# ckonst/VNDecorrelate

Hardware: AMD Instinct MI355X
Metric: Msamples/sec decorrelated (stereo, 30 taps) + achieved HBM GB/s vs roofline (higher is better)
Workload: dtype f32

## Files before the change

### vndecorrelate_amd/csrc/vnd_win.hpp

```cpp
#pragma once
#include "vnd_spec.hpp"
#include <cmath>
#include <functional>

namespace vnd {

static const char kWinKernelSource[] =
#include "vnd_win_kernel.inc"
    ;

struct WinGeom {
    int M = 0, nt = 0, G = 8;
    int C = 2;
    int DE = 0;
    int R = 0;
    int NB = 0;
    int plane = 0;
    int npl = 2;
    int tail = 0;
    int quad = 0;
    int split = 0;
    int nh() const { return split ? nt / 2 : (quad ? nt / (4 * quad) : nt); }
    int quad_pad() const { return quad == 2 ? 16 : 0; }
    size_t lds_bytes() const { return (size_t)(quad ? 2 * quad : 1) * (size_t)npl * (size_t)(M / 4) * (size_t)plane + (size_t)quad_pad(); }
// ... 76 lines not shown
                    if (j >= 1 && j <= M - 3) rd.ops.push_back(WinOp{1, (j - 1) / 2, h, tp.second, i});
                    else if (j == -1) rd.ops.push_back(WinOp{2, 0, h, tp.second, i});
                    else if (j == M - 1) rd.ops.push_back(WinOp{3, 0, h, tp.second, i});
                }
            }
        }
        if (!rd.ops.empty()) out.push_back(std::move(rd));
    }
    return out;
}

inline void win_traffic(const SpecTable &t, int M, size_t *lds_bytes, size_t *fmas)
{
    *lds_bytes = 0; *fmas = 0;
    for (int ch = 0; ch < t.C; ++ch) {
        *lds_bytes += 16 * win_schedule(t, ch, M).size();
        for (int32_t k = t.tap_off[ch]; k < t.tap_off[ch + 1]; ++k) if (t.w[k] != 0.0f) *fmas += (size_t)M;
    }
}

inline std::string win_taps_name(int pg) { return pg == 0 ? std::string("vw_taps") : "vw_taps_" + std::to_string(pg); }

inline std::string win_taps_channel_name(int pg, int ch)
{
    return pg == 0 ? "vw_taps_c" + std::to_string(ch) : "vw_taps_" + std::to_string(pg) + "c" + std::to_string(ch);
}

inline std::string win_taps_dispatch(const SpecTable &t)
{
    std::string s = "template <int PG> __device__ __forceinline__ void vw_taps_of(vw_lchar *const (&b)[2][VW_NBT], float (&o0)[VW_M], float (&o1)[VW_M])\n{\n";
    for (int pg = 0; pg < t.C / 2; ++pg)
        spec_append(s, "    %sif constexpr (PG == %d) %s(b, o0, o1);\n", pg ? "else " : "", pg, win_taps_name(pg).c_str());
    s += "}\n#define VW_DISPATCH(pg) switch (pg) {";
    for (int pg = 0; pg < t.C / 2; ++pg) spec_append(s, " case %d: vw_span<%d>(a, lds, stream, t_first, ntiles, flags, pace); break;", pg, pg);
    s += " default: break; }\n";
    return s;
}

inline std::string win_rd(const WinGeom &g, int ch, int o)
{
    const int dE = o / g.M, rr = (o % g.M) / 4;
    const int first_tail = g.R - g.nh() + 1;
    char buf[96];
    if (g.tail > 0 && dE >= first_tail) snprintf(buf, sizeof buf, "VW_RD(b[%d][%d], %d)", ch, g.NB + (dE - first_tail), rr * g.plane);
    else { const int kb = dE / g.G; snprintf(buf, sizeof buf, "VW_RD(b[%d][%d], %d)", ch, kb, (dE - kb * g.G) * 16 + rr * g.plane); }
    return buf;
}

inline bool win_adds_ok(const SpecTable &t)
{
    std::vector<float> mags;
    for (size_t k = 0; k < t.w.size(); ++k) {
        const float m = std::fabs(t.w[k]);
        if (m == 0.0f) continue;
        if (!std::isfinite(m) || m < 1e-18f || m > 1e18f) return false;
        if (std::find(mags.begin(), mags.end(), m) == mags.end()) mags.push_back(m);
        if (mags.size() > 8) return false;
    }
    for (int ch = 0; ch < t.C; ++ch) {
        std::vector<std::pair<int, float>> taps;
        for (int32_t k = t.tap_off[ch]; k < t.tap_off[ch + 1]; ++k)
            if (t.w[k] != 0.0f) taps.push_back({t.idx[k], std::fabs(t.w[k])});
        std::stable_sort(taps.begin(), taps.end(), [](const std::pair<int, float> &a, const std::pair<int, float> &b) { return a.first < b.first; });
        int changes = 0;
        for (size_t k = 1; k < taps.size(); ++k) changes += taps[k].second != taps[k - 1].second;
        if (changes > 8) return false;
    }
    return !mags.empty();
}

inline float win_unit_ratio(float from, float to) { return (float)((double)from / (double)to); }

inline void win_emit_adds_op(std::string &s, const std::string &acc, const std::string &x, bool pair, float w, float *unit)
{
    const float mag = std::fabs(w);
    const char sign = std::signbit(w) ? '-' : '+';
    if (*unit == 0.0f) spec_append(s, "    %s = %s %c %s;\n", acc.c_str(), pair ? "Z2" : "0.0f", sign, x.c_str());
    else if (*unit == mag) spec_append(s, "    %s = %s %c %s;\n", acc.c_str(), acc.c_str(), sign, x.c_str());
    else spec_append(s, "    %s = %s(%s, %s, %s%s);\n", acc.c_str(), pair ? "VW_FMA" : "__builtin_fmaf", acc.c_str(), spec_float(win_unit_ratio(*unit, mag)).c_str(),
                     sign == '-' ? "-" : "", x.c_str());
    *unit = mag;
}

template <class Name>
inline void win_emit_adds_merge(std::string &s, int ch, int M, const std::vector<float> &e_unit, const std::vector<float> &p_unit, float o0_unit, float ol_unit, Name name)
{
    float common = 0.0f;
    bool uniform = true;
    auto see = [&](float u) { if (u == 0.0f) return; if (common == 0.0f) common = u; else if (u != common) uniform = false; };
    for (float u : e_unit) see(u);
    for (float u : p_unit) see(u);
    see(o0_unit); see(ol_unit);
    for (int j = 0; j < M; ++j) {
        const float eu = e_unit[j / 2];
        const float ou = j == 0 ? o0_unit : (j == M - 1 ? ol_unit : p_unit[(j - 1) / 2]);
        std::string ev = eu != 0.0f ? (name(0, j / 2) + "." + ((j & 1) ? "y" : "x")) : std::string();
        std::string ov;
        if (ou != 0.0f) ov = j == 0 ? name(2, 0) : (j == M - 1 ? name(3, 0) : name(1, (j - 1) / 2) + "." + ((j & 1) ? "x" : "y"));
        if (!uniform) {
            if (!ev.empty()) ev = "(" + ev + " * " + spec_float(eu) + ")";
            if (!ov.empty()) ov = "(" + ov + " * " + spec_float(ou) + ")";
        }
        const std::string rhs = ev.empty() ? (ov.empty() ? std::string("0.0f") : ov) : (ov.empty() ? ev : ev + " + " + ov);
        spec_append(s, "    o%d[%d] = %s;\n", ch, j, rhs.c_str());
    }
    if (uniform && common != 0.0f && common != 1.0f) {
        const std::string u = spec_float(common);
        for (int k = 0; k < M / 2; ++k)
            spec_append(s, "    { const v2f t2 = v2f{o%d[%d], o%d[%d]} * v2f{%s, %s}; o%d[%d] = t2.x; o%d[%d] = t2.y; }\n", ch, 2 * k, ch, 2 * k + 1, u.c_str(), u.c_str(),
                        ch, 2 * k, ch, 2 * k + 1);
    }
}

inline std::string win_taps_function(const SpecTable &t, const WinGeom &g, int la, int pg = 0, int only_ch = -1, bool adds = false)
{
    const int M = g.M;
    std::string s;
    const std::string fname = only_ch < 0 ? win_taps_name(pg) : win_taps_channel_name(pg, only_ch);
    s += "__device__ __forceinline__ void " + fname + "(vw_lchar *const (&b)[2][VW_NBT], float (&o0)[VW_M], float (&o1)[VW_M])\n{\n";
    spec_append(s, "    v4f q[%d];\n    v2f E[%d], P[%d];\n    float O0, OL;\n", la + 1, M / 2, M / 2);
    if (adds) s += "    const v2f Z2 = {0.0f, 0.0f};\n";
    std::vector<WinRead> reads;
    size_t first_of_ch[3] = {0, 0, 0};
    for (int ch = 0; ch < 2; ++ch) {
        first_of_ch[ch] = reads.size();
        if (only_ch >= 0 && ch != only_ch) continue;
        std::vector<WinRead> one = win_schedule(t, 2 * pg + ch, M);
        std::reverse(one.begin(), one.end());
        if (adds)
            for (WinRead &r : one) std::stable_sort(r.ops.begin(), r.ops.end(), [](const WinOp &a, const WinOp &b) { return a.tap > b.tap; });
        for (WinRead &r : one) { r.ch = ch; reads.push_back(std::move(r)); }
    }
    first_of_ch[2] = reads.size();
    auto emit_read = [&](size_t k) {
        const WinRead &r = reads[k];
        spec_append(s, "    q[%zu] = %s;\n", k % (size_t)(la + 1), win_rd(g, r.ch, r.o).c_str());
    };
    auto emit_merge = [&](int ch, const std::vector<char> &e_used, const std::vector<char> &p_used, bool o0_used, bool ol_used) {
        for (int j = 0; j < M; ++j) {
            std::string ev = e_used[j / 2] ? ("E[" + std::to_string(j / 2) + "]." + ((j & 1) ? "y" : "x")) : std::string();
            std::string ov;
            if (j == 0) { if (o0_used) ov = "O0"; }
            else if (j == M - 1) { if (ol_used) ov = "OL"; }
            else if (p_used[(j - 1) / 2]) ov = "P[" + std::to_string((j - 1) / 2) + "]." + ((j & 1) ? "x" : "y");
            std::string rhs = ev.empty() ? (ov.empty() ? std::string("0.0f") : ov) : (ov.empty() ? ev : ev + " + " + ov);
            spec_append(s, "    o%d[%d] = %s;\n", ch, j, rhs.c_str());
        }
    };
    for (size_t k = 0; k < std::min(reads.size(), (size_t)la); ++k) emit_read(k);
    for (int ch = 0; ch < 2; ++ch) {
        if (only_ch >= 0 && ch != only_ch) continue;
        std::vector<char> e_used(M / 2, 0), p_used(M / 2, 0);
        bool o0_used = false, ol_used = false;
        std::vector<float> e_unit(M / 2, 0.0f), p_unit(M / 2, 0.0f);
        float o0_unit = 0.0f, ol_unit = 0.0f;
        for (size_t k = first_of_ch[ch]; k < first_of_ch[ch + 1]; ++k) {
            if (k + la < reads.size()) emit_read(k + la);
            const std::string qk = "q[" + std::to_string(k % (size_t)(la + 1)) + "]";
            for (const WinOp &op : reads[k].ops) {
                const std::string w = spec_float(op.w);
                if (adds) {
                    const bool pair = op.kind <= 1, is0 = op.kind == 2;
                    const std::string acc = pair ? std::string(op.kind == 0 ? "E[" : "P[") + std::to_string(op.acc) + "]" : std::string(is0 ? "O0" : "OL");
                    const std::string x = pair ? qk + (op.half ? ".zw" : ".xy") : qk + (is0 ? (op.half ? ".w" : ".y") : (op.half ? ".z" : ".x"));
                    win_emit_adds_op(s, acc, x, pair, op.w, pair ? (op.kind == 0 ? &e_unit[op.acc] : &p_unit[op.acc]) : (is0 ? &o0_unit : &ol_unit));
                    continue;
                }
                if (op.kind <= 1) {
                    const std::string acc = std::string(op.kind == 0 ? "E[" : "P[") + std::to_string(op.acc) + "]";
                    const std::string x = qk + (op.half ? ".zw" : ".xy");
                    char &used = op.kind == 0 ? e_used[op.acc] : p_used[op.acc];
                    if (used) spec_append(s, "    %s = VW_FMA(%s, %s, %s);\n", acc.c_str(), x.c_str(), w.c_str(), acc.c_str());
                    else spec_append(s, "    %s = VW_MUL(%s, %s);\n", acc.c_str(), x.c_str(), w.c_str());
                    used = 1;
                } else {
                    const bool is0 = op.kind == 2;
                    const std::string acc = is0 ? "O0" : "OL";
                    const std::string x = qk + (is0 ? (op.half ? ".w" : ".y") : (op.half ? ".z" : ".x"));
                    bool &used = is0 ? o0_used : ol_used;
                    if (used) spec_append(s, "    %s = __builtin_fmaf(%s, %s, %s);\n", acc.c_str(), x.c_str(), w.c_str(), acc.c_str());
                    else spec_append(s, "    %s = %s * %s;\n", acc.c_str(), x.c_str(), w.c_str());
                    used = true;
                }
            }
            s += "    VW_SB;\n";
        }
        if (adds)
            win_emit_adds_merge(s, ch, M, e_unit, p_unit, o0_unit, ol_unit, [](int kind, int k) {
                return kind == 0 ? "E[" + std::to_string(k) + "]" : (kind == 1 ? "P[" + std::to_string(k) + "]" : std::string(kind == 2 ? "O0" : "OL"));
            });
        else emit_merge(ch, e_used, p_used, o0_used, ol_used);
    }
    s += "}\n";
    return s;
}

struct WinExTap { int idx; float w; };
struct WinExPass { int ch; std::vector<WinExTap> taps; int end; float gain; };
struct WinExOp { int type, k; float w; };
struct WinExRead { int ch, o; size_t pass; std::vector<WinExOp> ops; };

inline std::vector<WinExPass> win_exact_passes(const SpecTable &t, int ch)
{
    std::vector<WinExPass> out;
    const int32_t k0 = t.tap_off[ch], k1 = t.tap_off[ch + 1];
    if (k0 == k1) return out;
    auto add_segment = [&](int32_t a, int32_t b, int end, float gain) {
        int32_t start = a;
        for (int32_t k = a + 1; k <= b; ++k) {
            if (k == b || t.idx[k] < t.idx[k - 1]) {
                WinExPass ps{ch, {}, k == b ? end : 0, gain};
                for (int32_t m = start; m < k; ++m) ps.taps.push_back(WinExTap{t.idx[m], t.w_raw[m]});
                out.push_back(std::move(ps));
                start = k;
            }
        }
    };
    if (!t.has_seg) {
        add_segment(k0, k1, 1, 1.0f);
    } else {
        int32_t prev = k0;
        for (int32_t sg = t.seg_off[ch]; sg < t.seg_off[ch + 1]; ++sg) {
            add_segment(prev, t.seg_end[sg], t.apply_gain ? 3 : 2, t.seg_gain[sg]);
            prev = t.seg_end[sg];
        }
    }
    return out;
}

inline void win_exact_reads(const std::vector<WinExPass> &passes, int M, std::vector<WinExRead> *reads, size_t pass_base)
{
    for (size_t p = 0; p < passes.size(); ++p) {
        const WinExPass &ps = passes[p];
        std::map<int, std::vector<WinExOp>> by_chunk;
        const bool singles = true;
        for (const WinExTap &tp : ps.taps) {
            if (singles && (tp.idx & 1)) {
                for (int j = -1; j < M; j += 2) {
                    const int e = tp.idx + j;
                    by_chunk[(e & 3) == 0 ? e : e - 2].push_back(WinExOp{((e & 3) == 0 ? 0 : 1) | 4, j, tp.w});
                }
                continue;
            }
            for (int j = 0; j < M; j += 2) {
                const int e = tp.idx + j;
                switch (e & 3) {
                case 0: by_chunk[e].push_back(WinExOp{0, j / 2, tp.w}); break;
                case 2: by_chunk[e - 2].push_back(WinExOp{1, j / 2, tp.w}); break;
                case 1: by_chunk[e - 1].push_back(WinExOp{3, j / 2, tp.w}); break;
                default: by_chunk[e + 1].push_back(WinExOp{2, j / 2, tp.w}); break;
                }
            }
        }
        std::vector<int> lend;
        for (const auto &kv : by_chunk)
            for (const WinExOp &op : kv.second)
                if (op.type == 2) { lend.push_back(kv.first - 4); break; }
        for (int o : lend) by_chunk[o];
        for (auto &kv : by_chunk) reads->push_back(WinExRead{ps.ch, kv.first, pass_base + p, std::move(kv.second)});
    }
}

inline void win_traffic_exact(const SpecTable &t, int M, size_t *lds_bytes, size_t *fmas)
{
    *lds_bytes = 0; *fmas = 0;
    for (int ch = 0; ch < t.C; ++ch) {
        std::vector<WinExRead> reads;
        const std::vector<WinExPass> passes = win_exact_passes(t, ch);
        if (!passes.empty()) win_exact_reads(passes, M, &reads, 0);
        *lds_bytes += 16 * reads.size();
        *fmas += (size_t)M * (size_t)(t.tap_off[ch + 1] - t.tap_off[ch]);
    }
}
// ... 430 lines not shown
```

### vndecorrelate_amd/csrc/vnd_win_kernel.inc

```
R"VNDWIN(
// vnd_spec_kernel, WINDOW form - the per-table tap sum with a register window (gfx950, wave64).
//
// Compiled at run time with hipRTC (vnd_win.hpp) behind a generated prologue that defines
//   VW_NT   threads per workgroup                 VW_M   consecutive output frames a lane owns per tile (16 | 32 | 64)
//   VW_R    ring entries (one entry = the M frames of one lane's run): NT of the tile + VW_DE of halo
//   VW_G    entries mirrored behind the ring, = the reach of one base register
//   VW_NB   base registers per channel (VW_DE / VW_G + 1)
//   VW_PLANE  bytes between the LDS planes of consecutive 16-byte chunks of an entry
//   VW_LA   LDS reads kept in flight ahead of the FMAs
//   VW_C    interleaved channels of the signal (even): a workgroup takes ONE channel pair of a span, 8 bytes of
//           every VW_C*4-byte frame (VW_C = 2: the whole frame, 16-byte accesses)
//   VW_Q    1: the QUAD form for signals of 4k channels - a workgroup takes a channel QUAD of a span (16 bytes of every
//           frame), a wave computes ONE channel of it (tap functions vw_taps_<pair>c<channel>) and stages and stores whole
//           16-byte pieces for all four (vw_span_qc below)
//           2: the OCTET form for signals of 8k channels - two neighbouring quads (32 bytes of every frame: with 8 channels,
//           whole frames and whole cache lines) per workgroup, an eighth of its lanes per channel
//   VW_S    1: the SPLIT form of a stereo signal - half the workgroup's waves compute channel 0, the others channel 1 (the tap
//           functions vw_taps_c0 / vw_taps_c1): a lane carries one channel's accumulators, so three waves fit a SIMD's registers
//           where the plain form holds two (vw_span_s below)
// and the functions vw_taps(), vw_taps_1(), ... (at the marker below): the tap sum of ONE lane for each channel
// pair, fully unrolled, with vw_taps_of<PG>() to pick one and VW_DISPATCH(pg): the span loop vw_span<pg> of a run-time pair number.
//
// The reference's tap sum (decorrelation.py:649-658, :402-414) asks, per output sample, for one input sample
// per tap.  vnd_spec_kernel.inc reads each of them from LDS (one aligned ds_read_b64 per tap and output
// ... 49 lines not shown
    // CHUNK of chunk_tiles consecutive tiles of one stream; the one dispatched first takes chunk_len0 of them, the next the rest
    // (chunk_tiles == 0: uniform spans, units walked as above)
    int chunk_tiles, chunk_len0, chunks_per_stream, cus_per_xcd;
    int stagger_ticks;       // a CU's second workgroup starts its prologue this many 100 MHz ticks after it enters the kernel
    int chunk_prio;          // 1: a CU's first-dispatched workgroup (the longer piece: the launch's critical path) runs at raised wave priority
    // BALANCED cut (stereo, uniform spans that would fill the resident workgroups unevenly): bal_total = streams x tiles_total > 0 - logical
    // workgroup L of nblocks walks the pool's tiles [L * bal_total / nblocks, (L + 1) * bal_total / nblocks), stream by stream: every
    // workgroup the same number of tiles (+- 1), a range that crosses into the next stream pays one more ring fill
    int bal_total;
    // VW_EPI, 32-frame runs: a wave's 64 runs are one 2048-frame block of the exact RMS sums (vnd_epilogue.hpp, rms_par_*): its sums of
    // squares of x and of the finished y, [stream][x0 x1 y0 y1][block] - the float64 PREDICTIONS the block-parallel sums start from
    // (every step of those is verified against the running sum: the values need not be the reference's, only close)
    double *epi_blk_sum;
    int epi_nblocks;
    int epi_rows_major;      // 1: [stream][block][x0 x1 y0 y1] instead - the rows epilogue_reduce_kernel adds up (the fused fast stage)
    // PACING of a CU's two co-resident workgroups (one round of persistent workgroups): the SIMDs issue the OLDER wave first, so the
    // workgroup publishes its count of finished tiles in its CU's slot pair and reads its partner's: the one BEHIND runs its next tile at
    // raised wave priority.  pace: [CU index][2] counters in device memory (never reset: a stale count only costs the first tile its bias)
    unsigned *pace;
};

struct VWPace { unsigned *mine; const unsigned *other; unsigned done; };

constexpr int VW_NW = VW_NT / 64;
constexpr int VW_QC = VW_M / 4;                 // 16-byte chunks per entry and channel
constexpr int VW_NH = VW_S ? VW_NT / 2 : VW_Q ? VW_NT / (4 * VW_Q) : VW_NT;  // lanes - and ring entries of a tile - per channel pair
constexpr int VW_T = VW_NH * VW_M;              // frames per tile
constexpr int VW_LPE = VW_Q ? VW_M * VW_Q : VW_M / 2;  // lanes of a 1 KB global access that fall into one entry (a lane moves a frame pair; VW_Q: one frame of four channels)
constexpr int VW_EPI_N = 64 / VW_LPE;           // entries per 1 KB global access
constexpr int VW_NI = VW_M / 2;                 // 1 KB global accesses per wave and tile
constexpr int VW_NPL = 2;                       // plane sets in LDS: one per output channel (the store phase transposes both channels' runs through them)
constexpr int VW_NXP = (VW_BC && !VW_S) ? 1 : 2; // ... of them holding INPUT: a mono input is staged once for both outputs (in the split form into both sets)
constexpr int VW_CH = VW_QC * VW_PLANE;         // byte offset of channel 1's planes
constexpr int VW_CX = VW_BC ? 1 : VW_C;         // interleaved INPUT channels
// channel pairs (VW_Q: quads or octets): one per workgroup and span.  4k + 2 channels (6, 10, ...) as QUADS: k full quads and one more that
// starts at channel C - 4 - it overlaps its neighbour in one channel pair, which both workgroups compute and write with the same bits
// (a frame's 16 bytes per access instead of the pair form's 8, for (k + 1) / (k + 1/2) of the arithmetic)
constexpr int VW_PAIRS = VW_Q ? (VW_C + 4 * VW_Q - 1) / (4 * VW_Q) : VW_C / 2;
constexpr int VW_PAIRB = 2 * VW_CH;             // VW_Q: byte offset of the second pair's plane sets
constexpr int VW_QUADB = 2 * VW_PAIRB + VW_QUADPAD; // octets: ... of the second QUAD's (shifted by 16 bytes: the two quads of a frame - neighbouring lanes of the 4-byte staging accesses - in different banks)
static_assert(VW_C >= 2 && VW_C % 2 == 0 && (VW_C == 2 || !VW_BC) && (VW_C == 2 || VW_Q || !VW_EPI), "whole channel pairs; fan-out and fused pointwise steps are stereo (quads / octets: the normaliser's sums only)");
static_assert(VW_Q == 0 || VW_Q == 1 || VW_Q == 2, "pairs, quads or octets");
static_assert(!VW_S || (VW_C == 2 && !VW_Q && !VW_EPI && VW_NT % 128 == 0 && VW_M >= 16), "split form: a stereo table, whole waves per channel");
static_assert(!VW_Q || ((VW_C % (4 * VW_Q) == 0 || (VW_Q == 1 && VW_C % 4 == 2 && VW_C >= 6)) && VW_NT % (256 * VW_Q) == 0 && VW_M * VW_Q <= 64 && VW_M <= 32), "quad / octet form: whole channel quads (4k + 2 channels: the last quad overlaps), whole waves per channel");
static_assert(VW_M == 16 || VW_M == 32 || VW_M == 64, "run length");
constexpr int VW_NBT = VW_NB + VW_TAIL;          // base registers per channel: the ring's, then one per entry offset that reaches into the tail
static_assert(VW_NT % 64 == 0 && VW_R >= VW_NH && VW_R + VW_TAIL == VW_NH + VW_DE && (VW_TAIL == 0 || (VW_Q && VW_R % 16 == 0)), "ring (+ tail) = tile + halo");
static_assert(VW_NB * VW_G > VW_DE, "bases cover the halo");
static_assert((VW_PLANE / 16) >= VW_R + VW_G + VW_TAIL, "plane stride: room for ring + mirror (+ tail)");
static_assert((VW_QC - 1) * VW_PLANE + VW_G * 16 < 65536 && VW_CH < 65536, "ds offset field is 16 bits");
static_assert((VW_Q ? 2 * VW_Q : 1) * VW_NPL * VW_QC * VW_PLANE + VW_QUADPAD <= 160 * 1024 && VW_QUADPAD % 16 == 0, "LDS");

// Raw buffer descriptor (stride 0): num_records = bytes left in the stream, so loads past the end of
// the stream return 0 (the reference's dropped terms, decorrelation.py:656-658) and stores past it
// are discarded.  Built from kernel arguments, blockIdx and the tile counter only: lives in SGPRs.
__device__ __forceinline__ v4i vw_rsrc(const void *base, long long bytes)
{
    const long long cap = 0x7fffffff;
    const unsigned long long addr = (unsigned long long)base;
    v4i r;
    r.x = (int)(unsigned)addr;
    r.y = (int)((unsigned)(addr >> 32) & 0xffffu);
    r.z = (int)(bytes < 0 ? 0 : (bytes > cap ? cap : bytes));
    r.w = 0x00020000;
    return r;
}

// blocks b and b + 8 share an XCD (and its L2): give one XCD consecutive logical ids, so that neighbouring
// spans (whose halos overlap) share an L2
__device__ __forceinline__ unsigned vw_xcd_remap(unsigned b, unsigned nwg)
{
    const unsigned q = nwg >> 3, r = nwg & 7u, xcd = b & 7u;
    const unsigned start = xcd < r ? xcd * (q + 1) : r * (q + 1) + (xcd - r) * q;
    return start + (b >> 3);
}

// (a mod R) for a < 2R, without a comparison: a - R wraps past 2^32 when a < R
__device__ __forceinline__ unsigned vw_wrap(unsigned a)
{
    const unsigned b = a - (unsigned)VW_R;
    return a < b ? a : b;
}

// one frame pair as {f0.c0, f0.c1, f1.c0, f1.c1}; a mono input fills the slots of channel 0.  In a wider signal the
// descriptor starts at the workgroup's channel pair: its 8 bytes of frames 2*pair and 2*pair + 1
__device__ __forceinline__ v4f vw_load_pair(v4i rsrc, int pair)
{
    if constexpr (VW_BC) {
        const v2f a = vw_load2(rsrc, pair * 8, 0, VW_LOAD_AUX);
        return v4f{a.x, 0.0f, a.y, 0.0f};
    } else if constexpr (VW_C == 2) {
        return vw_load4(rsrc, pair * 16, 0, VW_LOAD_AUX);
    } else {
        const v2f a = vw_load2(rsrc, pair * (VW_C * 8), 0, VW_LOAD_AUX), b = vw_load2(rsrc, pair * (VW_C * 8) + VW_C * 4, 0, VW_LOAD_AUX);
        return v4f{a.x, a.y, b.x, b.y};
    }
}

__device__ __forceinline__ void vw_store_pair(v4f v, v4i rsrc, int pair, int aux)
{
    if constexpr (VW_C == 2) {
        vw_store4(v, rsrc, pair * 16, 0, aux);
    } else {
        vw_store2(v2f{v.x, v.y}, rsrc, pair * (VW_C * 8), 0, aux);
        vw_store2(v2f{v.z, v.w}, rsrc, pair * (VW_C * 8) + VW_C * 4, 0, aux);
    }
}

// the staged pair goes to the channel planes (de-interleaved): 8 bytes each at `at` (chunk plane + entry + half)
__device__ __forceinline__ void vw_write_pair(vw_lchar *at, v4f v)
{
    *(vw_lv2f *)at = v2f{v.x, v.z};
    if constexpr (!VW_BC) *(vw_lv2f *)(at + VW_CH) = v2f{v.y, v.w};
}

#define VW_RD(base, imm) (*(const volatile vw_lv4f *)((base) + (imm)))
#define VW_FMA(x, w, a) __builtin_elementwise_fma((x), v2f{(w), (w)}, (a))
#define VW_MUL(x, w) ((x) * v2f{(w), (w)})
#define VW_SB __builtin_amdgcn_sched_barrier(0)
__device__ __forceinline__ float vw_add1(float a, float b)
{
    float r;
    asm("v_add_f32 %0, %1, %2" : "=v"(r) : "v"(a), "v"(b));
    return r;
}
__device__ __forceinline__ float vw_sub1(float a, float b)
{
    float r;
    asm("v_sub_f32 %0, %1, %2" : "=v"(r) : "v"(a), "v"(b));
    return r;
}
// (a.y, b.x) in ONE instruction: the exact mode's input pairs that start at an odd element (hipcc often takes two v_mov_b32)
__device__ __forceinline__ v2f vw_pair(v2f a, v2f b)
{
    v2f r;
    asm("v_pk_mov_b32 %0, %1, %2 op_sel:[1,0]" : "=v"(r) : "v"(a), "v"(b));
    return r;
}

//@@VW_TAPS@@

#if VW_STAMPS
// diagnosis (VND_WIN_STAMPS under VND_TUNING; tools/win_stamps.py): wave 0 of the first VW_STAMPS workgroups leaves the 100 MHz
// wall clock at its phase boundaries (first unit only) - [0] start, [1] ring filled, then for each of the first two tiles: taps done,
// (window dead: not kept), outputs exchanged, refill published; [14] the wave's stores acknowledged; [15] = HW_ID | XCC_ID << 32.  The stamps wait in SGPRs until the span is done
// (the kernel lives within a few VGPRs of its budget: a store per stamp made hipRTC's build spill).
__device__ unsigned long long vw_stamps[VW_STAMPS * 16];
#if VW_STAMP_PHASES
#define VW_STAMP_DECL unsigned vw_st[12] = {0, 0, 0, 0, 0, 0, 0, 0, 0, 0, 0, 0}
#define VW_STAMP(k) do { vw_st[k] = (unsigned)__builtin_amdgcn_s_memrealtime(); } while (0)
// ([12] = the workgroup's entry into the kernel, [13] = its exit (stores acknowledged), both written by the kernel function:
//  with VW_STAMP_PHASES 0 these two are all there is, and nothing is held in registers across the span)
#define VW_STAMP_FLUSH(on) do { if (on) { asm volatile("s_waitcnt vmcnt(0)" ::: "memory"); const unsigned long long end_ = __builtin_amdgcn_s_memrealtime(); if (threadIdx.x == VW_STAMP_WAVE * 64) { _Pragma("unroll") for (int q_ = 0; q_ < 12; ++q_) vw_stamps[blockIdx.x * 16 + q_] = vw_st[q_] ? (end_ - (unsigned long long)((unsigned)end_ - vw_st[q_])) : 0ull; vw_stamps[blockIdx.x * 16 + 14] = end_; } } } while (0)
#define VW_STAMP_TILE(t, k) do { if ((k) != 1 || VW_Q) { const unsigned now_ = (unsigned)__builtin_amdgcn_s_memrealtime(); _Pragma("unroll") for (int q_ = 0; q_ < 2; ++q_) if ((t) == q_) vw_st[2 + 4 * q_ + (k)] = now_; } } while (0)
#endif
#endif
#if !VW_STAMPS || !VW_STAMP_PHASES
#define VW_STAMP_DECL
#define VW_STAMP(k)
#define VW_STAMP_TILE(t, k)
#define VW_STAMP_FLUSH(on)
#endif

#if VW_EPI
// VelvetNoise.decorrelate's pointwise steps on one stereo frame, in the reference's float32 operation order
// (utils/dsp.py:59-63 side-channel encode, :34-37 stereo width; built with -ffp-contract=off)
__device__ __forceinline__ v2f vw_pointwise1(const VWArgs &a, v2f y, v2f x)          // one frame: {L, R}
{
    float y0 = y.x, y1 = y.y;
    if (a.epi_ms_encode) {
        const float mid = x.x + x.y;
        const float side = (y0 - y1) * 0.5f;
        y0 = (mid + side) * 0.5f;
        y1 = (mid - side) * 0.5f;
    }
    if (a.epi_use_width) {
        float m = (y0 + y1) * 0.5f, sd = (y0 - y1) * 0.5f;
        m = m * a.epi_w_mid;
        sd = sd * a.epi_w_side;
        y0 = m + sd;
        y1 = m - sd;
    }
    return v2f{y0, y1};
}
#endif

template <int PG>
__device__ __forceinline__ void vw_span(const VWArgs &a, vw_lchar *lds, long long stream, int t_first, int ntiles, int flags, VWPace &pace)
{
    const int tid = threadIdx.x;
    const int ln = tid & 63;
    const int wv = __builtin_amdgcn_readfirstlane(tid >> 6);
    const long long f0 = (long long)t_first * VW_T;
    // (the descriptors start at the channel pair: PGX / PG * 8 bytes into the first frame, and end as much before
    //  the end of the stream's last frame - inside the pair's last 8 bytes' frame, never in the next stream)
    constexpr int PGX = VW_BC ? 0 : PG;
// ... 397 lines not shown
        // With ONE wave per channel (NWH == 1: octets of 512 lanes, quads of 256) nobody else reads the channel's planes: the wave that
        // read the window is the one that overwrites it, in LDS program order - no barrier here, two per tile instead of three.
        if constexpr (NWH > 1) asm volatile("s_waitcnt lgkmcnt(0)\n\ts_barrier" ::: "memory");
        __builtin_amdgcn_s_setprio(1);
        vw_lchar *const mine = lp + (pc & 1) * VW_CH + pl * 16u;
#pragma unroll
        for (int r = 0; r < VW_QC; ++r)
            *(vw_lv4f *)(mine + r * VW_PLANE) = v4f{o[4 * r], o[4 * r + 1], o[4 * r + 2], o[4 * r + 3]};
        // X2. ... and the partner waves' (the other channels of the same 64 entries)
        asm volatile("s_waitcnt lgkmcnt(0)\n\ts_barrier" ::: "memory");
        VW_STAMP_TILE(t, 2);
        const long long fo = (long long)t * VW_T + (long long)we * VW_M;
        const v4i ry = vw_rsrc(ys + fo * VW_C, bytes_left - fo * FB);
        const long long fi = ((long long)(t + 1) * VW_NH + VW_R + we) * VW_M;
        const v4i rx = vw_rsrc(xs + fi * VW_C, bytes_need - fi * FB);
        constexpr int ST_AUX = VW_NT_STORES ? VW_NT_STORE_AUX : 0;
#pragma unroll
        for (int m = 0; m < NI; ++m) {
            vw_lchar *at = lds + lane_at + vw_wrap(pwl + (unsigned)(m * VW_EPI_N)) * 16u;
            const float c0 = *(const volatile vw_lfloat *)at, c1 = *(const volatile vw_lfloat *)(at + VW_CH);
            const float c2 = *(const volatile vw_lfloat *)(at + VW_PAIRB), c3 = *(const volatile vw_lfloat *)(at + VW_PAIRB + VW_CH);
            vw_store4(v4f{c0, c1, c2, c3}, ry, lg + m * (FPA * FB), 0, ST_AUX);
        }
        VW_STAMP_TILE(t, 1);                                                          // (quads / octets: read-backs and stores issued)
        const bool fin = (flags & 1) != 0 && t == ntiles - 1;          // (as vw_span: nothing to refill, nobody to wait for)
        if (!fin) {
            const bool mirror = pw < (unsigned)VW_G || pw + (unsigned)WE > (unsigned)VW_R;    // wave-uniform
#pragma unroll
            for (int m = 0; m < NI; ++m) {
                const unsigned e = vw_wrap(pwl + (unsigned)(m * VW_EPI_N));
                vw_lchar *at = lds + lane_at + e * 16u;
                vw_write_quad(at, pre[m]);
                if (mirror) { if (e < (unsigned)VW_G) vw_write_quad(at + VW_R * 16, pre[m]); }
                pre[m] = vw_load4(rx, lg + m * (FPA * FB), 0, VW_LOAD_AUX);
            }
#if VW_TAIL
            if (wv < NTA) {                                                              // wave-uniform
                const unsigned e = (unsigned)(wv * VW_EPI_N) + (unsigned)lane_e;
                if (e < (unsigned)VW_TAIL) vw_write_quad(lds + lane_at + ((unsigned)(VW_R + VW_G) + e) * 16u, tailreg);      // tile t + 1's
                const long long ft = ((long long)(t + 2) * VW_NH + VW_R + wv * VW_EPI_N) * VW_M;                               // tile t + 2's
                tailreg = vw_load4(vw_rsrc(xs + ft * VW_C, bytes_need - ft * FB), lg, 0, VW_LOAD_AUX);
            }
#endif
        }
        p0 = p0 + VW_NH >= VW_R ? p0 + VW_NH - VW_R : p0 + VW_NH;
        __builtin_amdgcn_s_setprio(0);
        if (!fin) asm volatile("s_waitcnt lgkmcnt(0)\n\ts_barrier" ::: "memory");
        VW_STAMP_TILE(t, 3);
    }
    VW_STAMP_FLUSH(vw_stamp_on);
}
#endif

#if VW_S
// ---- the SPLIT form of a stereo signal: a wave computes ONE channel ---------------------------------------
// The plain form's lane carries both channels' work one after the other: E / P accumulators, the first channel's finished
// outputs and a tile of prefetched frames - ~240 registers, two waves per SIMD.  Here waves 0 .. NW/2-1 run channel 0's tap
// function (vw_taps_c0) on the tile's NT/2 entries and the other half channel 1's: per lane one channel's accumulators, half
// the prefetch - three waves per SIMD fit (two workgroups of 384 lanes per CU: 12 waves), on the same ring and the same
// 1 KB global accesses.  A frame's two channels now sit in two waves: outputs go as planar runs into the tile's dead
// entries, one barrier more, then each wave reads back and stores the 32 entries it also refills (as vw_span_qc).
template <int CH>
__device__ __forceinline__ void vw_taps_ch(vw_lchar *const (&b)[2][VW_NBT], float (&o)[VW_M])
{
    if constexpr (CH == 0) vw_taps_c0(b, o, o);
    else vw_taps_c1(b, o, o);
}

__device__ __forceinline__ void vw_span_s(const VWArgs &a, vw_lchar *lds, long long stream, int t_first, int ntiles, int flags, VWPace &pace)
{
    constexpr int NWH = VW_NW / 2;                                       // waves per channel
    constexpr int NI = VW_M / 4;                                         // 1 KB global STORES per wave and tile (64 frame pairs each)
    // VW_BC - a mono input fanned out: the one input channel is staged into BOTH plane sets (each output channel's waves read their own
    // copy with the tap functions of the stereo form unchanged), 16 bytes = 4 frames per lane and access: half as many input accesses,
    // each 256 frames = 256 / M ring entries (stereo: 128 frames)
    constexpr int NIN = VW_BC ? VW_M / 8 : VW_M / 4;                     // 1 KB global LOADS per wave and tile
    constexpr int EIN = VW_BC ? 256 / VW_M : VW_EPI_N;                   // ring entries per load
    constexpr int XB = VW_BC ? 4 : 8;                                    // input bytes per frame
    // the refill's frames: NE accesses are prefetched a tile ahead and held in registers through the tap phase, the other
    // LATE are loaded at the start of the store phase that consumes them (64-frame runs: the accumulators need the room)
    constexpr int LATE = VW_LATE < NIN ? VW_LATE : NIN - 1;
    constexpr int NE = NIN - LATE;
    static_assert(VW_LATE >= 0 && LATE < NIN, "late refill accesses");
    const int tid = threadIdx.x;
    const int ln = tid & 63;
    const int wv = __builtin_amdgcn_readfirstlane(tid >> 6);
    const int pc = wv >= NWH ? 1 : 0;                                    // the wave's channel
    const int wl = wv - pc * NWH;
    const int tl = wl * 64 + ln;                                         // the entry of a tile this LANE computes (in its channel)
    const int we = wl * 64 + pc * 32;                                    // the first of the 32 entries this WAVE stages and stores (both channels)
    const long long f0 = (long long)t_first * VW_T;
    const float *xs = a.x + (stream * a.n + f0) * (XB / 4);
    float *ys = a.y + (stream * a.n + f0) * 2;
    const long long bytes_left = (a.n - f0) * 8;                         // (of the output)
    const long long need = ((long long)ntiles * VW_T + (long long)VW_DE * VW_M) * XB;
    const long long bytes_need = need < (a.n - f0) * XB ? need : (a.n - f0) * XB;
#if VW_LANE_SWIZZLE
    const int lq = (ln & ~24) | ((ln & 8) << 1) | ((ln & 16) >> 1);      // (as vw_span: the 8-byte staging writes and read-backs touch every bank once)
#else
    const int lq = ln;
#endif
    const int lane_e = lq / VW_LPE;
    const int lane_at = ((lq % VW_LPE) >> 1) * VW_PLANE + (lq & 1) * 8;
    // ... and in a 1 KB LOAD: stereo as above; mono - 4 frames = one 16-byte chunk of entry ln / (M / 4), written to both plane sets
    const int in_e = VW_BC ? ln / (VW_M / 4) : lane_e;
    const int in_at = VW_BC ? (ln % (VW_M / 4)) * VW_PLANE : lane_at;
    const int in16 = VW_BC ? ln * 16 : lq * 16;                          // the lane's byte offset in a load
    auto stage = [&](vw_lchar *at, v4f v) {
        if constexpr (VW_BC) { *(vw_lv4f *)at = v; *(vw_lv4f *)(at + VW_CH) = v; }
        else vw_write_pair(at, v);
    };
#if VW_STAMPS && VW_STAMP_PHASES
    const bool vw_stamp_on = blockIdx.x < VW_STAMPS && (a.chunk_tiles > 0 || a.bal_total > 0 || (unsigned)(stream * a.spans + t_first / a.tiles_per_span) == vw_xcd_remap(blockIdx.x, a.nblocks));
    if (vw_stamp_on && threadIdx.x == 0) {
        unsigned hw, xcc;
        asm volatile("s_getreg_b32 %0, hwreg(HW_REG_HW_ID)" : "=s"(hw));
        asm volatile("s_getreg_b32 %0, hwreg(HW_REG_XCC_ID)" : "=s"(xcc));
        vw_stamps[blockIdx.x * 16 + 15] = (unsigned long long)hw | ((unsigned long long)xcc << 32);
    }
#endif
    VW_STAMP_DECL;
    VW_STAMP(0);

    {
        const v4i rx = vw_rsrc(xs, bytes_need);
        constexpr int NFILL = (VW_R + EIN - 1) / EIN;
        constexpr int PER = (NFILL + VW_NW - 1) / VW_NW;
        constexpr int BATCH = 8;
        for (int k0 = 0; k0 < PER; k0 += BATCH) {
            v4f w[BATCH];
#pragma unroll
            for (int kk = 0; kk < BATCH; ++kk) {
                const int i = wv + VW_NW * (k0 + kk);
                w[kk] = vw_load4(rx, i * 1024 + in16, 0, VW_LOAD_AUX);
            }
#pragma unroll
            for (int kk = 0; kk < BATCH; ++kk) {
                const int i = wv + VW_NW * (k0 + kk);
                const int e = i * EIN + in_e;
                if (k0 + kk < PER && e < VW_R) {
                    stage(lds + in_at + e * 16, w[kk]);
                    if (e < VW_G) stage(lds + in_at + (e + VW_R) * 16, w[kk]);
                }
            }
        }
    }
    v4f pre[NE];
    {
        const long long f = ((long long)VW_R + we) * VW_M;
        const v4i rx = vw_rsrc(xs + f * (XB / 4), bytes_need - f * XB);
#pragma unroll
        for (int m = 0; m < NE; ++m) pre[m] = vw_load4(rx, 1024 * m + in16, 0, VW_LOAD_AUX);
    }
    asm volatile("s_waitcnt lgkmcnt(0)\n\ts_barrier" ::: "memory");
    VW_STAMP(1);
    bool hi = (flags & 2) != 0;                                          // (wave-uniform) raised priority: a chunk's first workgroup - or, paced, the one behind
    if (hi) __builtin_amdgcn_s_setprio(2);

    unsigned p0 = 0;
    for (int t = 0; t < ntiles; ++t) {
        // the last tile of the workgroup's last unit refills nothing: no loads, no staging writes, no barrier behind its stores
        const bool fin = (flags & 1) != 0 && t == ntiles - 1;
        const unsigned pw = vw_wrap(p0 + (unsigned)we);
        const unsigned pl = vw_wrap(p0 + (unsigned)tl);
        // (a lane's byte offset in a 1 KB access and its entry in it, made opaque per tile: hipcc otherwise hoists the sums with
        //  64-frame runs is what spilled)
        int lq16 = lq * 16, in16o = in16;
        unsigned pwl = pw + (unsigned)lane_e, pwi = pw + (unsigned)in_e;
        asm volatile("" : "+v"(lq16), "+v"(pwl));
        if constexpr (VW_BC) asm volatile("" : "+v"(in16o), "+v"(pwi));
        float o[VW_M];
        {
            vw_lchar *b[2][VW_NBT];
#pragma unroll
            for (int k = 0; k < VW_NB; ++k) {
                b[0][k] = lds + vw_wrap(pl + (unsigned)(k * VW_G)) * 16u;
                b[1][k] = b[0][k] + VW_CH;
            }
            if (pc == 0) vw_taps_ch<0>(b, o);
            else vw_taps_ch<1>(b, o);
        }
#pragma unroll
        for (int j = 0; j < VW_M; ++j) asm volatile("" : "+v"(o[j]));
        VW_STAMP_TILE(t, 0);
        // X. every wave is done reading this tile's window: the tile's own entries are dead (both channels)
        asm volatile("s_waitcnt lgkmcnt(0)\n\ts_barrier" ::: "memory");
        VW_STAMP_TILE(t, 1);
        if (hi) __builtin_amdgcn_s_setprio(3);
        else __builtin_amdgcn_s_setprio(1);
        // (pacing: the partner's count, in flight through the store phase)
        unsigned seen = 0;
        if (pace.other != nullptr) seen = __hip_atomic_load(pace.other, __ATOMIC_RELAXED, __HIP_MEMORY_SCOPE_AGENT);
        // (the late part of THIS tile's refill: in flight through the transposition and the stores)
        v4f late[LATE > 0 ? LATE : 1];
        if constexpr (LATE > 0) {                                        // (also on a final tile: out of range there, no data moves)
            const long long fl = ((long long)t * VW_NH + VW_R + we) * VW_M;
            const v4i rl = vw_rsrc(xs + fl * (XB / 4), bytes_need - fl * XB);
#pragma unroll
            for (int m = 0; m < LATE; ++m) late[m] = vw_load4(rl, (VW_BC ? in16o : lq16) + 1024 * (NE + m), 0, VW_LOAD_AUX);
        }
        // the lane's run into its own dead entry, planar (its channel's planes)
        vw_lchar *const mine = lds + pc * VW_CH + pl * 16u;
#pragma unroll
        for (int r = 0; r < VW_QC; ++r)
            *(vw_lv4f *)(mine + r * VW_PLANE) = v4f{o[4 * r], o[4 * r + 1], o[4 * r + 2], o[4 * r + 3]};
        // X2. ... and the partner wave's (the other channel of the same 64 entries)
        asm volatile("s_waitcnt lgkmcnt(0)\n\ts_barrier" ::: "memory");
        VW_STAMP_TILE(t, 2);
        const long long fo = (long long)t * VW_T + (long long)we * VW_M;
        const v4i ry = vw_rsrc(ys + fo * 2, bytes_left - fo * 8);
        const long long fi = ((long long)(t + 1) * VW_NH + VW_R + we) * VW_M;
        const v4i rx = vw_rsrc(xs + fi * (XB / 4), bytes_need - fi * XB);
        constexpr int ST_AUX = VW_NT_STORES ? VW_NT_STORE_AUX : 0;
        //  short launch nothing much, covers these round trips: tools/ablate/RUNS.md: run_r4c, run_r4g.sh)
#pragma unroll
        for (int m = 0; m < NI; ++m) {
            vw_lchar *at = lds + lane_at + vw_wrap(pwl + (unsigned)(m * VW_EPI_N)) * 16u;
            const v2f r0 = *(const volatile vw_lv2f *)at, r1 = *(const volatile vw_lv2f *)(at + VW_CH);
            vw_store4(v4f{r0.x, r1.x, r0.y, r1.y}, ry, lq16 + 1024 * m, 0, ST_AUX);
        }
        if (!fin) {
            const bool mirror = pw < (unsigned)VW_G || pw + 32u > (unsigned)VW_R;             // wave-uniform
#pragma unroll
            for (int m = 0; m < NIN; ++m) {
                const unsigned e = vw_wrap((VW_BC ? pwi : pwl) + (unsigned)(m * EIN));
                vw_lchar *at = lds + in_at + e * 16u;
                const v4f v = m < NE ? pre[m < NE ? m : 0] : late[m >= NE ? m - NE : 0];
                stage(at, v);
                if (mirror) { if (e < (unsigned)VW_G) stage(at + VW_R * 16, v); }
                if (m < NE) pre[m < NE ? m : 0] = vw_load4(rx, (VW_BC ? in16o : lq16) + 1024 * m, 0, VW_LOAD_AUX);
            }
        }
        p0 = p0 + VW_NH >= VW_R ? p0 + VW_NH - VW_R : p0 + VW_NH;
        pace.done += 1;
        if (pace.other != nullptr) {
            if (threadIdx.x == 0) __hip_atomic_store(pace.mine, pace.done, __ATOMIC_RELAXED, __HIP_MEMORY_SCOPE_AGENT);
            hi = (unsigned)__builtin_amdgcn_readfirstlane((int)seen) > pace.done;       // the partner is ahead: this workgroup's next tile goes first
        }
        if (hi) __builtin_amdgcn_s_setprio(2);
        else __builtin_amdgcn_s_setprio(0);
        // Y. the refill is in place for every wave's window
        if (!fin) asm volatile("s_waitcnt lgkmcnt(0)\n\ts_barrier" ::: "memory");
        VW_STAMP_TILE(t, 3);
    }
    if (hi) __builtin_amdgcn_s_setprio(0);
    VW_STAMP_FLUSH(vw_stamp_on);
}
#endif

// VW_WAVES_PER_EU: the waves per SIMD that the LDS footprint and the registers let a CU hold - as minimum AND maximum:
// the scheduler must not trade registers for an occupancy the LDS will not grant
extern "C" __global__ __launch_bounds__(VW_NT) __attribute__((amdgpu_waves_per_eu(VW_WAVES_PER_EU, VW_WAVES_PER_EU)))
void vnd_spec_kernel(const VWArgs a)
{
#if VW_STAMPS
    { const unsigned long long entry_ = __builtin_amdgcn_s_memrealtime(); if (threadIdx.x == 0 && blockIdx.x < VW_STAMPS) vw_stamps[blockIdx.x * 16 + 12] = entry_; }
#endif
    extern __shared__ __attribute__((aligned(16))) float lds_generic[];
    vw_lchar *lds = (vw_lchar *)(vw_lfloat *)lds_generic;
    // One round of workgroups: more units than resident slots are walked inside the kernel
    // (the channel pairs of a span are neighbouring units: their workgroups touch the same lines at about the same time)
    const unsigned first = vw_xcd_remap(blockIdx.x, a.nblocks);
    // (ONE call site of the span loop - it is the whole tap sum, inlined - for both ways of cutting the work)
    const bool chunked = VW_PAIRS == 1 && a.chunk_tiles > 0;
    VWPace pace = {nullptr, nullptr, 0u};
    if (a.pace != nullptr && !chunked) {
        // the CU this workgroup runs on (HW_ID: cu 11:8, sh 12, se 15:13; XCC_ID) and its dispatch round there
        unsigned hw, xcc;
        asm volatile("s_getreg_b32 %0, hwreg(HW_REG_HW_ID)" : "=s"(hw));
        asm volatile("s_getreg_b32 %0, hwreg(HW_REG_XCC_ID)" : "=s"(xcc));
        const unsigned cu = (((xcc & 7u) * 8u + ((hw >> 13) & 7u)) * 2u + ((hw >> 12) & 1u)) * 16u + ((hw >> 8) & 15u);
        const unsigned round = ((blockIdx.x >> 3) / (unsigned)a.cus_per_xcd) & 1u;
        pace.mine = a.pace + cu * 2u + round;
        pace.other = a.pace + cu * 2u + (round ^ 1u);
        if (threadIdx.x == 0) __hip_atomic_store(pace.mine, 0u, __ATOMIC_RELAXED, __HIP_MEMORY_SCOPE_AGENT);
    }
    const bool balanced = VW_PAIRS == 1 && !chunked && a.bal_total > 0;
    long long g = 0, g_end = 0;                                          // balanced: this workgroup's range of the pool's tiles
    if (balanced) {
        g = (long long)first * a.bal_total / (long long)a.nblocks;
        g_end = (long long)(first + 1u) * a.bal_total / (long long)a.nblocks;
    }
    for (unsigned unit = first; chunked || (balanced ? g < g_end : unit < a.units); unit += a.nblocks) {
        int pg = 0, t_first, ntiles;
        long long stream;
        if (balanced) {
            stream = g / a.tiles_total;
            t_first = (int)(g - stream * a.tiles_total);
            const long long left_s = a.tiles_total - t_first, left_w = g_end - g;
            ntiles = (int)(left_s < left_w ? left_s : left_w);
            g += ntiles;
        } else if (chunked) {
            // HW_ID, tools/win_stamps.py): workgroup j of XCD x runs on CU j mod cus_per_xcd as that CU's (j / cus_per_xcd)-th.  Were the
            // dispatch ever different, every piece would still be computed exactly once - only the balance would suffer.
            const unsigned xcd = blockIdx.x & 7u, j = blockIdx.x >> 3;
            const unsigned cu = j % (unsigned)a.cus_per_xcd, round = j / (unsigned)a.cus_per_xcd;
            const unsigned g = xcd * (unsigned)a.cus_per_xcd + cu;                           // the CU's chunk
            stream = g / (unsigned)a.chunks_per_stream;
            const int chunk = (int)(g % (unsigned)a.chunks_per_stream);
            const int len = round == 0 ? a.chunk_len0 : (round == 1 ? a.chunk_tiles - a.chunk_len0 : 0);
            t_first = chunk * a.chunk_tiles + (round == 0 ? 0 : a.chunk_len0);
            const int left = a.tiles_total - t_first;
            ntiles = left < len ? left : len;
            if (ntiles <= 0) break;
            if (round != 0 && a.stagger_ticks > 0) {
                const unsigned long long until = __builtin_amdgcn_s_memrealtime() + (unsigned long long)a.stagger_ticks;
                while (__builtin_amdgcn_s_memrealtime() < until) __builtin_amdgcn_s_sleep(8);
            }
        } else {
            unsigned id = unit;
            pg = (int)(id % (unsigned)VW_PAIRS);
            id /= (unsigned)VW_PAIRS;
// ... 18 lines not shown
```

Baseline: 698,600.

## Compute ring LDS addresses from wave-uniform parts and use packed moves for swizzles

Ring addresses for store and load accesses are now built from a wave-uniform first entry computed on the scalar unit plus one per-lane constant. This replaces per-lane wrap arithmetic, and the mirror test becomes scalar compares. Channel swizzles use v_pk_mov_b32 via inline asm instead of pairs of v_mov. Channel-1 LDS bases are made opaque so the compiler does not fold large offsets into each read. The aim is fewer VALU instructions per tile in the memory-bound store and refill phases. The cost is more complex edge-case logic at the ring end and the mirror region.

```diff
diff --git a/vndecorrelate_amd/csrc/vnd_win.hpp b/vndecorrelate_amd/csrc/vnd_win.hpp
--- a/vndecorrelate_amd/csrc/vnd_win.hpp
+++ b/vndecorrelate_amd/csrc/vnd_win.hpp
@@ -182,8 +182,13 @@
     *unit = mag;
 }
 
+inline std::string win_merge_sum(const std::string &ev, const std::string &ov, bool single)
+{
+    return single ? "vw_add1(" + ev + ", " + ov + ")" : ev + " + " + ov;
+}
+
 template <class Name>
-inline void win_emit_adds_merge(std::string &s, int ch, int M, const std::vector<float> &e_unit, const std::vector<float> &p_unit, float o0_unit, float ol_unit, Name name)
+inline void win_emit_adds_merge(std::string &s, int ch, int M, const std::vector<float> &e_unit, const std::vector<float> &p_unit, float o0_unit, float ol_unit, Name name, bool single = false)
 {
     float common = 0.0f;
     bool uniform = true;
@@ -201,7 +206,7 @@
             if (!ev.empty()) ev = "(" + ev + " * " + spec_float(eu) + ")";
             if (!ov.empty()) ov = "(" + ov + " * " + spec_float(ou) + ")";
         }
-        const std::string rhs = ev.empty() ? (ov.empty() ? std::string("0.0f") : ov) : (ov.empty() ? ev : ev + " + " + ov);
+        const std::string rhs = ev.empty() ? (ov.empty() ? std::string("0.0f") : ov) : (ov.empty() ? ev : win_merge_sum(ev, ov, single));
         spec_append(s, "    o%d[%d] = %s;\n", ch, j, rhs.c_str());
     }
     if (uniform && common != 0.0f && common != 1.0f) {
@@ -243,7 +248,7 @@
             if (j == 0) { if (o0_used) ov = "O0"; }
             else if (j == M - 1) { if (ol_used) ov = "OL"; }
             else if (p_used[(j - 1) / 2]) ov = "P[" + std::to_string((j - 1) / 2) + "]." + ((j & 1) ? "x" : "y");
-            std::string rhs = ev.empty() ? (ov.empty() ? std::string("0.0f") : ov) : (ov.empty() ? ev : ev + " + " + ov);
+            std::string rhs = ev.empty() ? (ov.empty() ? std::string("0.0f") : ov) : (ov.empty() ? ev : win_merge_sum(ev, ov, g.split != 0));
             spec_append(s, "    o%d[%d] = %s;\n", ch, j, rhs.c_str());
         }
     };
@@ -288,7 +293,7 @@
         if (adds)
             win_emit_adds_merge(s, ch, M, e_unit, p_unit, o0_unit, ol_unit, [](int kind, int k) {
                 return kind == 0 ? "E[" + std::to_string(k) + "]" : (kind == 1 ? "P[" + std::to_string(k) + "]" : std::string(kind == 2 ? "O0" : "OL"));
-            });
+            }, g.split != 0);
         else emit_merge(ch, e_used, p_used, o0_used, ol_used);
     }
     s += "}\n";
diff --git a/vndecorrelate_amd/csrc/vnd_win_kernel.inc b/vndecorrelate_amd/csrc/vnd_win_kernel.inc
--- a/vndecorrelate_amd/csrc/vnd_win_kernel.inc
+++ b/vndecorrelate_amd/csrc/vnd_win_kernel.inc
@@ -155,6 +155,25 @@
     return a < b ? a : b;
 }
 
+// instructions: written in C, hipcc spells either half with single v_mov_b32 - about six per 16-byte access of the store phase
+__device__ __forceinline__ v2f vw_lows(v2f a, v2f b)
+{
+    v2f r;
+    asm("v_pk_mov_b32 %0, %1, %2 op_sel:[0,0]" : "=v"(r) : "v"(a), "v"(b));
+    return r;
+}
+__device__ __forceinline__ v2f vw_highs(v2f a, v2f b)
+{
+    v2f r;
+    asm("v_pk_mov_b32 %0, %1, %2 op_sel:[1,1]" : "=v"(r) : "v"(a), "v"(b));
+    return r;
+}
+__device__ __forceinline__ v4f vw_zip(v2f a, v2f b)
+{
+    const v2f lo = vw_lows(a, b), hi = vw_highs(a, b);
+    return v4f{lo.x, lo.y, hi.x, hi.y};
+}
+
 // one frame pair as {f0.c0, f0.c1, f1.c0, f1.c1}; a mono input fills the slots of channel 0.  In a wider signal the
 // descriptor starts at the workgroup's channel pair: its 8 bytes of frames 2*pair and 2*pair + 1
 __device__ __forceinline__ v4f vw_load_pair(v4i rsrc, int pair)
@@ -183,8 +202,8 @@
 // the staged pair goes to the channel planes (de-interleaved): 8 bytes each at `at` (chunk plane + entry + half)
 __device__ __forceinline__ void vw_write_pair(vw_lchar *at, v4f v)
 {
-    *(vw_lv2f *)at = v2f{v.x, v.z};
-    if constexpr (!VW_BC) *(vw_lv2f *)(at + VW_CH) = v2f{v.y, v.w};
+    *(vw_lv2f *)at = vw_lows(v2f{v.x, v.y}, v2f{v.z, v.w});
+    if constexpr (!VW_BC) *(vw_lv2f *)(at + VW_CH) = vw_highs(v2f{v.x, v.y}, v2f{v.z, v.w});
 }
 
 #define VW_RD(base, imm) (*(const volatile vw_lv4f *)((base) + (imm)))
@@ -748,6 +767,20 @@
     constexpr int LATE = VW_LATE < NIN ? VW_LATE : NIN - 1;
     constexpr int NE = NIN - LATE;
     static_assert(VW_LATE >= 0 && LATE < NIN, "late refill accesses");
+    // RING ADDRESSES FROM WAVE-UNIFORM PARTS.  A wave's 32 entries start at pw, and access m of it takes the EPI_N (a store) or EIN (a
+    // load) entries from pw + m x that number on: the FIRST of them is wave-uniform - scalar arithmetic - and a lane adds ONE constant
+    // (its entry within the access, its chunk plane and half): one v_add_u32 per access.  That needs the entries of an access to stay
+    // together at the ring's end and at the mirror's:
+    //   * the ring's length and G multiples of their number - the ring advances by whole tiles (NH entries, a multiple of 64) and a wave
+    //     starts 32 entries into one, so every access then starts at a multiple too; or
+    //   * entry PAIRS (64-frame runs) on any ring: the pair that starts at the ring's last entry has its second half at entry 0 (the
+    //     lanes' other constant, picked by a scalar compare), and whether a lane's entry has a mirror - all of the pair below G - 1,
+    //     the first half at G - 1, the second at R - 1 - is a scalar compare and a fixed half of the wave.
+    // (Any other ring: per lane, as vw_span)
+    constexpr bool UNI_O = VW_EPI_N == 2 || VW_R % VW_EPI_N == 0;
+    constexpr bool UNI_I = EIN == 2 || (VW_R % EIN == 0 && VW_G % EIN == 0);
+    constexpr bool ENDS_O = VW_R % VW_EPI_N != 0, ENDS_I = VW_R % EIN != 0;      // an access can straddle the ring's end (pairs only)
+    static_assert(VW_NH % 64 == 0 && 32 % VW_EPI_N == 0 && 32 % EIN == 0, "a wave's accesses start at whole multiples of their entries");
     const int tid = threadIdx.x;
     const int ln = tid & 63;
     const int wv = __builtin_amdgcn_readfirstlane(tid >> 6);
@@ -772,9 +805,26 @@
     const int in_e = VW_BC ? ln / (VW_M / 4) : lane_e;
     const int in_at = VW_BC ? (ln % (VW_M / 4)) * VW_PLANE : lane_at;
     const int in16 = VW_BC ? ln * 16 : lq * 16;                          // the lane's byte offset in a load
+    // UNI_O / UNI_I: all of a lane's own in the LDS address of a store / load access, and (_w) where the access straddles the ring's end
+    int lane_c = lane_e * 16 + lane_at, lane_cw = lane_c - lane_e * (VW_R * 16), in_c = in_e * 16 + in_at, in_cw = in_c - in_e * (VW_R * 16);
+    asm volatile("" : "+v"(lane_c), "+v"(lane_cw));                      // (ONE register each: hipcc would take the sums apart again)
+    if constexpr (VW_BC) asm volatile("" : "+v"(in_c), "+v"(in_cw));
+    else { in_c = lane_c; in_cw = lane_cw; }
     auto stage = [&](vw_lchar *at, v4f v) {
         if constexpr (VW_BC) { *(vw_lv4f *)at = v; *(vw_lv4f *)(at + VW_CH) = v; }
         else vw_write_pair(at, v);
+    };
+    // ... and, where the entry has one, into its mirror as well: the pair is taken apart once
+    auto stage_both = [&](vw_lchar *at, v4f v, bool mirrored) {
+        if constexpr (VW_BC) {
+            stage(at, v);
+            if (mirrored) stage(at + VW_R * 16, v);
+        } else {
+            const v2f c0 = vw_lows(v2f{v.x, v.y}, v2f{v.z, v.w}), c1 = vw_highs(v2f{v.x, v.y}, v2f{v.z, v.w});
+            *(vw_lv2f *)at = c0;
+            *(vw_lv2f *)(at + VW_CH) = c1;
+            if (mirrored) { *(vw_lv2f *)(at + VW_R * 16) = c0; *(vw_lv2f *)(at + VW_R * 16 + VW_CH) = c1; }
+        }
     };
 #if VW_STAMPS && VW_STAMP_PHASES
     const bool vw_stamp_on = blockIdx.x < VW_STAMPS && (a.chunk_tiles > 0 || a.bal_total > 0 || (unsigned)(stream * a.spans + t_first / a.tiles_per_span) == vw_xcd_remap(blockIdx.x, a.nblocks));
@@ -829,12 +879,21 @@
         const bool fin = (flags & 1) != 0 && t == ntiles - 1;
         const unsigned pw = vw_wrap(p0 + (unsigned)we);
         const unsigned pl = vw_wrap(p0 + (unsigned)tl);
-        // (a lane's byte offset in a 1 KB access and its entry in it, made opaque per tile: hipcc otherwise hoists the sums with
+        // (a lane's byte offset in a 1 KB access and, per lane, its entry in it, made opaque per tile: hipcc otherwise hoists the sums
         //  64-frame runs is what spilled)
         int lq16 = lq * 16, in16o = in16;
         unsigned pwl = pw + (unsigned)lane_e, pwi = pw + (unsigned)in_e;
-        asm volatile("" : "+v"(lq16), "+v"(pwl));
-        if constexpr (VW_BC) asm volatile("" : "+v"(in16o), "+v"(pwi));
+        asm volatile("" : "+v"(lq16));
+        if constexpr (!UNI_O || (!UNI_I && !VW_BC)) asm volatile("" : "+v"(pwl));
+        if constexpr (VW_BC) asm volatile("" : "+v"(in16o));
+        if constexpr (VW_BC && !UNI_I) asm volatile("" : "+v"(pwi));
+        // byte offset in a plane of the lane's part of store access m
+        auto out_at = [&](int m) -> unsigned {
+            if constexpr (UNI_O) {
+                const unsigned es = vw_wrap(pw + (unsigned)(m * VW_EPI_N));
+                return es * 16u + (unsigned)((ENDS_O && es == (unsigned)(VW_R - 1)) ? lane_cw : lane_c);
+            } else return vw_wrap(pwl + (unsigned)(m * VW_EPI_N)) * 16u + (unsigned)lane_at;
+        };
         float o[VW_M];
         {
             vw_lchar *b[2][VW_NBT];
@@ -844,7 +903,13 @@
                 b[1][k] = b[0][k] + VW_CH;
             }
             if (pc == 0) vw_taps_ch<0>(b, o);
-            else vw_taps_ch<1>(b, o);
+            else {
+                // (channel 1 reads through ITS bases: left to hipcc, their VW_CH is folded into every read's offset instead, and the
+                //  chunk planes that lands beyond the 16-bit offset field get an address add per read)
+#pragma unroll
+                for (int k = 0; k < VW_NB; ++k) asm volatile("" : "+v"(b[1][k]));
+                vw_taps_ch<1>(b, o);
+            }
         }
 #pragma unroll
         for (int j = 0; j < VW_M; ++j) asm volatile("" : "+v"(o[j]));
@@ -881,19 +946,28 @@
         //  short launch nothing much, covers these round trips: tools/ablate/RUNS.md: run_r4c, run_r4g.sh)
 #pragma unroll
         for (int m = 0; m < NI; ++m) {
-            vw_lchar *at = lds + lane_at + vw_wrap(pwl + (unsigned)(m * VW_EPI_N)) * 16u;
+            vw_lchar *at = lds + out_at(m);
             const v2f r0 = *(const volatile vw_lv2f *)at, r1 = *(const volatile vw_lv2f *)(at + VW_CH);
-            vw_store4(v4f{r0.x, r1.x, r0.y, r1.y}, ry, lq16 + 1024 * m, 0, ST_AUX);
+            vw_store4(vw_zip(r0, r1), ry, lq16 + 1024 * m, 0, ST_AUX);
         }
         if (!fin) {
-            const bool mirror = pw < (unsigned)VW_G || pw + 32u > (unsigned)VW_R;             // wave-uniform
+            // (wave-uniform; UNI_I: every access asks for itself, on the scalar unit - one loop, not a copy of it per answer)
+            const bool mirror = pw < (unsigned)VW_G || pw + 32u > (unsigned)VW_R;
 #pragma unroll
             for (int m = 0; m < NIN; ++m) {
-                const unsigned e = vw_wrap((VW_BC ? pwi : pwl) + (unsigned)(m * EIN));
-                vw_lchar *at = lds + in_at + e * 16u;
+                // (UNI_I: the access's first entry - scalar - else the lane's)
+                const unsigned e = vw_wrap((UNI_I ? pw : (VW_BC ? pwi : pwl)) + (unsigned)(m * EIN));
+                vw_lchar *at = lds + e * 16u + (unsigned)(UNI_I ? ((ENDS_I && e == (unsigned)(VW_R - 1)) ? in_cw : in_c) : in_at);
                 const v4f v = m < NE ? pre[m < NE ? m : 0] : late[m >= NE ? m - NE : 0];
-                stage(at, v);
-                if (mirror) { if (e < (unsigned)VW_G) stage(at + VW_R * 16, v); }
+                if constexpr (UNI_I) {
+                    bool mirrored = e + (unsigned)EIN <= (unsigned)VW_G;
+                    if constexpr (VW_G % EIN != 0 || ENDS_I) mirrored = mirrored || (e == (unsigned)(VW_G - 1) && in_e == 0);   // (a pair that starts at an odd entry)
+                    if constexpr (ENDS_I) mirrored = mirrored || (e == (unsigned)(VW_R - 1) && in_e == 1);
+                    stage_both(at, v, mirrored);
+                } else {
+                    stage(at, v);
+                    if (mirror) { if (e < (unsigned)VW_G) stage(at + VW_R * 16, v); }
+                }
                 if (m < NE) pre[m < NE ? m : 0] = vw_load4(rx, (VW_BC ? in16o : lq16) + 1024 * m, 0, VW_LOAD_AUX);
             }
         }
```

Result: no change. 701,000 (median of 3 runs) (+0.3%).
